# m4rch1n0/vqvae

Hardware: AMD Instinct MI355X
Metric: latents/sec through geodesic kNN+APSP+K-medoids (higher is better)
Workload: dtype f64-exact(u32 fixed point)

## Files before the change

vqvae_amd/csrc/common.hip:

```cpp
#include "geo_common.h"

#include <cstdlib>
#include <cstring>

namespace geo {

namespace {
struct OptionName { const char *name, *env; int Options::*field; };
const OptionName kOptionNames[] = {
    {"sssp_sb", "GEO_SSSP_SB", &Options::sssp_sb},
    {"sssp_act", "GEO_SSSP_ACT", &Options::sssp_act},
    {"sssp_sparse_div", "GEO_SSSP_SPARSE_DIV", &Options::sssp_sparse_div},
    {"sssp_map_div", "GEO_SSSP_MAP_DIV", &Options::sssp_map_div},
    {"sssp_group", "GEO_SSSP_GROUP", &Options::sssp_group},
    {"sssp_grouped_cap", "GEO_SSSP_GROUPED_CAP", &Options::sssp_grouped_cap},
    {"sssp_trace", "GEO_SSSP_TRACE", &Options::sssp_trace},
    {"sssp_u32", "GEO_SSSP_U32", &Options::sssp_u32},
    {"sssp_push", "GEO_SSSP_PUSH", &Options::sssp_push},
    {"sssp_order", "GEO_SSSP_ORDER", &Options::sssp_order},
    {"sssp_delta", "GEO_SSSP_DELTA", &Options::sssp_delta},
    {"sssp_push_blocks", "GEO_SSSP_PUSH_BLOCKS", &Options::sssp_push_blocks},
    {"knn_filter", "GEO_KNN_FILTER", &Options::knn_filter},
    {"kpp_grid", "GEO_KPP_GRID", &Options::kpp_grid},
    {"kpp_profile", "GEO_KPP_PROFILE", &Options::kpp_profile},
    {"jvp_mid", "GEO_JVP_MID", &Options::jvp_mid},
    {"jvp_back_valu", "GEO_JVP_BACK_VALU", &Options::jvp_back_valu},
    {"jvp_front_valu", "GEO_JVP_FRONT_VALU", &Options::jvp_front_valu},
    {"jvp_per_node", "GEO_JVP_PER_NODE", &Options::jvp_per_node},
    {"jvp_node_jacobian", "GEO_JVP_NODE_JACOBIAN", &Options::jvp_node_jacobian},
    {"jvp_start_dedup", "GEO_JVP_START_DEDUP", &Options::jvp_start_dedup},
    {"jvp_front_once", "GEO_JVP_FRONT_ONCE", &Options::jvp_front_once},
};
Options from_environment() {
    Options o;
    for (const OptionName &e : kOptionNames) {
        const char *v = getenv(e.env);
        if (!v) continue;
        if (e.field == &Options::jvp_mid) o.jvp_mid = v[0] == 'c' ? 2 : (v[0] == 'a' ? 3 : atoi(v));
        else o.*(e.field) = atoi(v);
    }
    return o;
}
}

Options &options() {
    static Options o = from_environment();
    return o;
}

static thread_local char g_err[512] = "";

void set_error(const char *fmt, ...) {
    va_list ap;
    va_start(ap, fmt);
    vsnprintf(g_err, sizeof(g_err), fmt, ap);
    va_end(ap);
}

constexpr int SCAN_THREADS = 256;
constexpr int SCAN_ITEMS = 8;
constexpr int SCAN_TILE = SCAN_THREADS * SCAN_ITEMS;

__global__ __launch_bounds__(SCAN_THREADS) void scan_tiles_kernel(const int32_t *__restrict__ in,
                                                                 int32_t *__restrict__ out,
                                                                 int32_t *__restrict__ tile_sums, int64_t n) {
    __shared__ int32_t wave_tot[SCAN_THREADS / 64];
    const int64_t base = (int64_t)blockIdx.x * SCAN_TILE + (int64_t)threadIdx.x * SCAN_ITEMS;
    int32_t v[SCAN_ITEMS];
    int32_t run = 0;
#pragma unroll
    for (int i = 0; i < SCAN_ITEMS; ++i) {
        int32_t x = (base + i < n) ? in[base + i] : 0;
        v[i] = run;
        run += x;
    }
    const int lane = threadIdx.x & 63, wave = threadIdx.x >> 6;
    int32_t inc = run;
#pragma unroll
    for (int off = 1; off < 64; off <<= 1) {
        int32_t t = __shfl_up(inc, off, 64);
        if (lane >= off) inc += t;
    }
    if (lane == 63) wave_tot[wave] = inc;
    __syncthreads();
    int32_t wave_base = 0, total = 0;
#pragma unroll
    for (int w = 0; w < SCAN_THREADS / 64; ++w) {
        if (w < wave) wave_base += wave_tot[w];
        total += wave_tot[w];
    }
    const int32_t excl = wave_base + inc - run;
#pragma unroll
    for (int i = 0; i < SCAN_ITEMS; ++i)
        if (base + i < n) out[base + i] = excl + v[i];
    if (threadIdx.x == 0) tile_sums[blockIdx.x] = total;
}

__global__ __launch_bounds__(SCAN_THREADS) void scan_add_kernel(int32_t *__restrict__ out,
                                                               const int32_t *__restrict__ tile_offs, int64_t n,
                                                               int64_t n_tiles) {
    const int64_t base = (int64_t)blockIdx.x * SCAN_TILE + (int64_t)threadIdx.x * SCAN_ITEMS;
    const int32_t add = tile_offs[blockIdx.x];
#pragma unroll
    for (int i = 0; i < SCAN_ITEMS; ++i)
        if (base + i < n) out[base + i] += add;
    if (blockIdx.x == 0 && threadIdx.x == 0) out[n] = tile_offs[n_tiles];
}

__global__ void scan_single_total_kernel(int32_t *out, const int32_t *tile_sums, int64_t n) {
    if (threadIdx.x == 0 && blockIdx.x == 0) out[n] = tile_sums[0];
}

static int64_t tiles_of(int64_t n) { return (n + SCAN_TILE - 1) / SCAN_TILE; }

size_t scan_tmp_bytes(int64_t n) {
    size_t total = 0;
    int64_t m = n;
    while (true) {
        int64_t t = tiles_of(m > 0 ? m : 1);
        total += align_up((size_t)(t + 1) * sizeof(int32_t)) * 2;
        if (t <= 1) break;
        m = t;
    }
    return total + 256;
}

static int scan_rec(const int32_t *in, int32_t *out, int64_t n, Arena &ar, hipStream_t s) {
    const int64_t t = tiles_of(n > 0 ? n : 1);
    int32_t *sums = ar.take<int32_t>((size_t)t + 1);
    int32_t *offs = ar.take<int32_t>((size_t)t + 1);
    if (!sums || !offs) {
        set_error("exclusive_scan: workspace too small");
        return GEO_E_WORKSPACE;
    }
    scan_tiles_kernel<<<dim3((unsigned)t), dim3(SCAN_THREADS), 0, s>>>(in, out, sums, n);
    GEO_LAUNCH_CHECK();
    if (t == 1) {
        scan_single_total_kernel<<<1, 64, 0, s>>>(out, sums, n);
        GEO_LAUNCH_CHECK();
        return GEO_OK;
    }
    int rc = scan_rec(sums, offs, t, ar, s);
    if (rc != GEO_OK) return rc;
    scan_add_kernel<<<dim3((unsigned)t), dim3(SCAN_THREADS), 0, s>>>(out, offs, n, t);
    GEO_LAUNCH_CHECK();
    return GEO_OK;
}

int exclusive_scan_i32(const int32_t *in, int32_t *out, int64_t n, void *tmp, size_t tmp_bytes,
                       int64_t *total_host, hipStream_t stream) {
    Arena ar(tmp, tmp_bytes);
    int rc = scan_rec(in, out, n, ar, stream);
    if (rc != GEO_OK) return rc;
    if (total_host) {
        int32_t tot = 0;
        GEO_HIP_CHECK(hipMemcpyAsync(&tot, out + n, sizeof(int32_t), hipMemcpyDeviceToHost, stream));
        GEO_HIP_CHECK(hipStreamSynchronize(stream));
        *total_host = tot;
    }
    return GEO_OK;
}

}

extern "C" int geo_version(void) { return 109; }
extern "C" const char *geo_last_error(void) { return geo::g_err; }

extern "C" int geo_set_option(const char *name, int32_t value) {
    if (name)
        for (const geo::OptionName &e : geo::kOptionNames)
            if (strcmp(name, e.name) == 0) {
                geo::options().*(e.field) = value;
                return GEO_OK;
            }
    geo::set_error("geo_set_option: unknown option '%s'", name ? name : "(null)");
    return GEO_E_ARG;
}
```

vqvae_amd/csrc/geo_common.h:

```cpp
#pragma once
#include <hip/hip_runtime.h>

#include <cstdarg>
#include <cstdint>
#include <cstdio>

#include "geo_hip.h"

namespace geo {

void set_error(const char *fmt, ...);

#define GEO_HIP_CHECK(expr)                                                                      \
    do {                                                                                         \
        hipError_t _e = (expr);                                                                  \
        if (_e != hipSuccess) {                                                                  \
            geo::set_error("%s failed: %s (%s:%d)", #expr, hipGetErrorString(_e), __FILE__, __LINE__); \
            return GEO_E_HIP;                                                                    \
        }                                                                                        \
    } while (0)

#define GEO_REQUIRE(cond, ...)              \
    do {                                    \
        if (!(cond)) {                      \
            geo::set_error(__VA_ARGS__);    \
            return GEO_E_ARG;               \
        }                                   \
    } while (0)

#define GEO_LAUNCH_CHECK() GEO_HIP_CHECK(hipGetLastError())

struct Options {
    int sssp_sb = -1, sssp_act = 1, sssp_sparse_div = -1, sssp_map_div = -1, sssp_group = 1, sssp_grouped_cap = 256,
        sssp_trace = 0, sssp_u32 = 1, sssp_push = 1 ,
        sssp_delta = 8 , sssp_order = 0 , sssp_push_blocks = 64, knn_filter = 1, kpp_grid = 256, kpp_profile = 0, jvp_mid = 0 ,
        jvp_back_valu = 0, jvp_front_valu = 0, jvp_per_node = 1 ,
        jvp_node_jacobian = 1 ,
        jvp_start_dedup = 1 ,
        jvp_front_once = 1 ;
};
Options &options();

static inline size_t align_up(size_t x, size_t a = 256) { return (x + a - 1) / a * a; }

struct Arena {
    char *base;
    size_t size, off;
    Arena(void *p, size_t n) : base(static_cast<char *>(p)), size(n), off(0) {}
    template <typename T>
    T *take(size_t count) {
        size_t bytes = align_up(count * sizeof(T));
        if (off + bytes > size) return nullptr;
        T *r = reinterpret_cast<T *>(base + off);
        off += bytes;
        return r;
    }
};

size_t scan_tmp_bytes(int64_t n);
int exclusive_scan_i32(const int32_t *in, int32_t *out, int64_t n, void *tmp, size_t tmp_bytes,
                       int64_t *total_host, hipStream_t stream);

static inline int grid_for(int64_t work_items, int per_block, int cap = 8192) {
    int64_t g = (work_items + per_block - 1) / per_block;
    if (g < 1) g = 1;
    if (g > cap) g = cap;
    return static_cast<int>(g);
}

}
```

vqvae_amd/csrc/jvp.hip:

```cpp
#include "geo_common.h"

#include <cmath>
#include <cstdlib>
#include <type_traits>
#include <vector>

namespace {

constexpr int TS = 32;
constexpr int NC = 128;
constexpr int MAX_BLOCKS = 4;
constexpr int FRONT_MAX_N1 = 1024;
constexpr int BACK_TS = 8;

typedef float f32x16 __attribute__((ext_vector_type(16)));
typedef __bf16 bf16x8 __attribute__((ext_vector_type(8)));
typedef unsigned short u16x8 __attribute__((ext_vector_type(8)));

struct Shape {
    int d, c0, c1, c2, co, s_out, pad3, p_out;
    int n1, n2;
    int opix_per_chunk, n_chunks;
};

// ... 1521 lines not shown
#pragma unroll
                for (int part = 0; part < 3; ++part) {
                    if (MODE != 1) *reinterpret_cast<u16x8 *>(&A3[part][0][ss][k0 + k8]) = pp[part];
                    if (MODE != 2) *reinterpret_cast<u16x8 *>(&A3[part][1][ss][k0 + k8]) = pt[part];
                }
            }
        }
        __syncthreads();
#pragma unroll
        for (int kq = 0; kq < 2; ++kq) {
            const int ks = wave * 2 + kq;
            bf16x8 ap[3], at[3];
#pragma unroll
            for (int part = 0; part < 3; ++part) {
                if (MODE != 1) ap[part] = *reinterpret_cast<const bf16x8 *>(&A3[part][0][r][ks * 16 + h * 8]);
                if (MODE != 2) at[part] = *reinterpret_cast<const bf16x8 *>(&A3[part][1][r][ks * 16 + h * 8]);
            }
#pragma unroll
            for (int nt = 0; nt < NT; ++nt) {
                bf16x8 b[3];
#pragma unroll
                for (int part = 0; part < 3; ++part)
                    b[part] = *reinterpret_cast<const bf16x8 *>(
                        W3b + ((((size_t)kb * 3 + part) * 8 + ks) * 2 + h) * (size_t)NP * 8 + (size_t)(nt * 32 + r) * 8);
                if (MODE != 1) accp[nt] = __builtin_amdgcn_mfma_f32_32x32x16_bf16(ap[2], b[0], accp[nt], 0, 0, 0);
                if (MODE != 2) acct[nt] = __builtin_amdgcn_mfma_f32_32x32x16_bf16(at[2], b[0], acct[nt], 0, 0, 0);
                if (MODE != 1) accp[nt] = __builtin_amdgcn_mfma_f32_32x32x16_bf16(ap[0], b[2], accp[nt], 0, 0, 0);
                if (MODE != 2) acct[nt] = __builtin_amdgcn_mfma_f32_32x32x16_bf16(at[0], b[2], acct[nt], 0, 0, 0);
                if (MODE != 1) accp[nt] = __builtin_amdgcn_mfma_f32_32x32x16_bf16(ap[1], b[1], accp[nt], 0, 0, 0);
                if (MODE != 2) acct[nt] = __builtin_amdgcn_mfma_f32_32x32x16_bf16(at[1], b[1], acct[nt], 0, 0, 0);
                if (MODE != 1) accp[nt] = __builtin_amdgcn_mfma_f32_32x32x16_bf16(ap[1], b[0], accp[nt], 0, 0, 0);
                if (MODE != 2) acct[nt] = __builtin_amdgcn_mfma_f32_32x32x16_bf16(at[1], b[0], acct[nt], 0, 0, 0);
                if (MODE != 1) accp[nt] = __builtin_amdgcn_mfma_f32_32x32x16_bf16(ap[0], b[1], accp[nt], 0, 0, 0);
                if (MODE != 2) acct[nt] = __builtin_amdgcn_mfma_f32_32x32x16_bf16(at[0], b[1], acct[nt], 0, 0, 0);
                if (MODE != 1) accp[nt] = __builtin_amdgcn_mfma_f32_32x32x16_bf16(ap[0], b[0], accp[nt], 0, 0, 0);
                if (MODE != 2) acct[nt] = __builtin_amdgcn_mfma_f32_32x32x16_bf16(at[0], b[0], acct[nt], 0, 0, 0);
            }
        }
    }
    float *red = reinterpret_cast<float *>(&A3[0][0][0][0]);
    const int row = threadIdx.x >> 3, c4 = (threadIdx.x & 7) * 4;
    const size_t nrow = MODE == 1 ? (row_map ? (size_t)row_map[slot0 + row] : node_of(row)) : slot0 + row;
    float *jrow = nullptr;
    if (MODE == 1 && jac_node) {
        const int64_t e = edge_of(row);
        if (e >= 0) jrow = jac_node + (nrow * unit_d + (size_t)(e % unit_d)) * NP;
    }
    double sumsq = 0.0;
#pragma unroll
    for (int nt = 0; nt < NT; ++nt) {
        __syncthreads();
#pragma unroll
        for (int q = 0; q < 16; ++q) {
            const int rr = (q & 3) + 8 * (q >> 2) + 4 * (lane >> 5);
            if (MODE != 1) red[((wave * 2 + 0) * 32 + rr) * 33 + (lane & 31)] = accp[nt][q];
            if (MODE != 2) red[((wave * 2 + 1) * 32 + rr) * 33 + (lane & 31)] = acct[nt][q];
        }
        __syncthreads();
#pragma unroll
        for (int c = 0; c < 4; ++c) {
            const int o = nt * 32 + c4 + c;
            if (o < P) {
                float x = b3[o / (s_out * s_out)], t = 0.f;
#pragma unroll
                for (int w = 0; w < 4; ++w) {
                    if (MODE != 1) x += red[((w * 2 + 0) * 32 + row) * 33 + c4 + c];
                    if (MODE != 2) t += red[((w * 2 + 1) * 32 + row) * 33 + c4 + c];
                }
                const float sg = MODE == 1 ? sg_node[nrow * NP + o] : 1.0f / (1.0f + expf(-x));
                if (MODE == 2) sg_node[nrow * NP + o] = sg;
                const float j = t * sg * (1.0f - sg);
                if (MODE == 1 && jrow) jrow[o] = j;
                sumsq += (double)(j * j);
            }
        }
    }
    sumsq += __shfl_xor(sumsq, 1, 64);
    sumsq += __shfl_xor(sumsq, 2, 64);
    sumsq += __shfl_xor(sumsq, 4, 64);
    if (MODE != 2 && (threadIdx.x & 7) == 0) norms[slot0 + row] = (float)sqrt(sumsq);
    }
}

__global__ __launch_bounds__(256) void combine_kernel(const float *__restrict__ norms, int64_t e_base, int64_t e_count,
                                                     int batch, int slots_per_group, float *__restrict__ len_out) {
    for (int64_t i = (int64_t)blockIdx.x * blockDim.x + threadIdx.x; i < e_count; i += (int64_t)gridDim.x * blockDim.x) {
        const int64_t chunk = i / batch, within = i % batch;
        const float a = norms[(chunk * 2 + 0) * slots_per_group + within];
        const float b = norms[(chunk * 2 + 1) * slots_per_group + within];
        len_out[e_base + i] = 0.5f * (a + b);
    }
}

__global__ __launch_bounds__(256) void pair_edges_kernel(int64_t n_nodes, int d, int64_t n_pseudo, int32_t *__restrict__ src,
                                                        int32_t *__restrict__ dst) {
    for (int64_t i = (int64_t)blockIdx.x * blockDim.x + threadIdx.x; i < n_pseudo; i += (int64_t)gridDim.x * blockDim.x) {
        const int64_t a = 2 * (i / d), b = a + 1 < n_nodes ? a + 1 : n_nodes - 1;
        src[i] = (int32_t)a;
        dst[i] = (int32_t)b;
    }
}

__global__ __launch_bounds__(256) void jacobian_lengths_kernel(const float *__restrict__ z, const int32_t *__restrict__ src,
                                                              const int32_t *__restrict__ dst, int64_t n_edges, int d, int p_out,
                                                              int np, const float *__restrict__ jac_node,
                                                              float *__restrict__ len_out) {
    const int64_t gid = (int64_t)blockIdx.x * 256 + threadIdx.x;
    const int l = (int)(gid & 15);
    int64_t e = gid >> 4;
    const bool live = e < n_edges;
    if (!live) e = n_edges - 1;
    const int64_t a = src[e], b = dst[e];
    float dz[16];
#pragma unroll
    for (int k = 0; k < 16; ++k) dz[k] = k < d ? z[b * d + k] - z[a * d + k] : 0.f;
    float end_norm[2];
#pragma unroll
    for (int side = 0; side < 2; ++side) {
        const float *J = jac_node + (size_t)(side ? b : a) * d * np;
        double sumsq = 0.0;
        for (int o = l; o < p_out; o += 16) {
            float v = 0.f;
#pragma unroll
            for (int k = 0; k < 16; ++k)
                if (k < d) v = fmaf(dz[k], J[(size_t)k * np + o], v);
            sumsq += (double)(v * v);
        }
        sumsq += __shfl_xor(sumsq, 1, 64);
        sumsq += __shfl_xor(sumsq, 2, 64);
        sumsq += __shfl_xor(sumsq, 4, 64);
        sumsq += __shfl_xor(sumsq, 8, 64);
        end_norm[side] = (float)sqrt(sumsq);
    }
    if (live && l == 0) len_out[e] = 0.5f * (end_norm[0] + end_norm[1]);
}

bool make_shape(const geo_decoder_desc *dc, Shape *s) {
    s->d = dc->latent_dim; s->c0 = dc->c0; s->c1 = dc->c1; s->c2 = dc->c2; s->co = dc->out_channels;
    if (dc->out_size == 28) { s->s_out = 4; s->pad3 = 3; }
    else if (dc->out_size == 32) { s->s_out = 8; s->pad3 = 1; }
    else return false;
    s->p_out = s->co * s->s_out * s->s_out;
    s->n1 = 4 * s->c1; s->n2 = 16 * s->c2;
    if (s->c2 <= 0 || NC % s->c2 != 0) return false;
    if (s->c1 <= 0 || 4 * s->c1 > FRONT_MAX_N1) return false;
    s->opix_per_chunk = NC / s->c2;
    if (s->opix_per_chunk > 16) s->opix_per_chunk = 16;
    s->n_chunks = 16 / s->opix_per_chunk;
    return true;
}

void make_chunks(const Shape &s, ChunkTable *t) {
    static const int order[16][2] = {{0, 1}, {0, 2}, {3, 1}, {3, 2}, {1, 0}, {2, 0}, {1, 3}, {2, 3},
                                     {1, 1}, {1, 2}, {2, 1}, {2, 2}, {0, 0}, {0, 3}, {3, 0}, {3, 3}};
    for (int ch = 0; ch < 16; ++ch) { t->nblk[ch] = 0; for (int i = 0; i < 16; ++i) t->opix[ch][i] = 0; }
    for (int ch = 0; ch < s.n_chunks; ++ch) {
        bool used[4] = {false, false, false, false};
        for (int lo = 0; lo < s.opix_per_chunk; ++lo) {
            const int oy = order[ch * s.opix_per_chunk + lo][0], ox = order[ch * s.opix_per_chunk + lo][1];
            t->opix[ch][lo] = oy * 4 + ox;
            for (int iy = 0; iy < 2; ++iy)
                for (int ix = 0; ix < 2; ++ix) {
                    const int ky = oy + 1 - 2 * iy, kx = ox + 1 - 2 * ix;
                    if (ky >= 0 && ky < 4 && kx >= 0 && kx < 4) used[iy * 2 + ix] = true;
                }
        }
        for (int ip = 0; ip < 4; ++ip)
            if (used[ip]) t->ipix[ch][t->nblk[ch]++] = ip;
    }
}

bool chunks_match_mid_geom(const ChunkTable &tab, int *bad_chunk) {
    for (int ch = 0; ch < 8; ++ch) {
        int nb = 0;
        bool ok = true;
        for (int ip = 0; ip < 4; ++ip) {
            const int blk = MidGeom::blk_of(ch, ip);
            if (blk >= 0) { ok = ok && tab.ipix[ch][blk] == ip; ++nb; }
        }
        ok = ok && nb == tab.nblk[ch] && tab.opix[ch][0] == MidGeom::opix(ch, 0) && tab.opix[ch][1] == MidGeom::opix(ch, 1);
        if (!ok) { *bad_chunk = ch; return false; }
    }
    return true;
}

struct Plan {
    Shape sh;
    int batch, tiles_per_group, slots_per_group;
    int64_t chunks_per_pass;
    size_t bytes;
    size_t pass_slots() const { return (size_t)chunks_per_pass * 2 * slots_per_group; }
};

constexpr int64_t MAX_SLOTS_PER_PASS = 1 << 20;

size_t round_up_to_tile(int64_t n) { return n > 0 ? ((size_t)n + TS - 1) / TS * TS : 0; }

size_t node_bytes(const Shape &s, int64_t n_nodes) {
    if (n_nodes <= 0) return 0;
    const size_t np = (size_t)((s.p_out + 31) / 32) * 32;
    return geo::align_up(round_up_to_tile(n_nodes) * s.n2 * 4) + geo::align_up(round_up_to_tile(n_nodes) * np * 4);
}

bool make_plan(const geo_decoder_desc *dc, int64_t n_edges, int batch, Plan *p) {
    if (!make_shape(dc, &p->sh)) return false;
    p->batch = batch;
    p->tiles_per_group = (batch + TS - 1) / TS;
    p->slots_per_group = p->tiles_per_group * TS;
    const int64_t chunks = (n_edges + batch - 1) / batch;
    int64_t cpp = MAX_SLOTS_PER_PASS / (2 * (int64_t)p->slots_per_group);
    if (cpp < 1) cpp = 1;
    if (cpp > chunks) cpp = chunks > 0 ? chunks : 1;
    p->chunks_per_pass = cpp;
    const Shape &s = p->sh;
    const size_t slots = p->pass_slots(), tiles = slots / TS, groups = (size_t)cpp * 2;
    size_t b = 0;
    b += geo::align_up((size_t)s.d * s.n1 * 4) + geo::align_up((size_t)s.n1 * 4);
    b += geo::align_up((size_t)s.n_chunks * MAX_BLOCKS * s.c1 * NC * 4);
    b += geo::align_up((size_t)s.n_chunks * MAX_BLOCKS * s.c1 * NC * 2 * 3);
    b += geo::align_up((size_t)16 * s.co * s.c2 * 4);
    b += geo::align_up((size_t)16 * s.c2 * 192 * 3 * 2);
    b += 2 * geo::align_up(slots * s.n1 * 4) + 2 * geo::align_up(slots * s.n2 * 4);
    b += geo::align_up(tiles * s.n1 * 4 * 8) + geo::align_up(tiles * s.n2 * 4 * 8);
    b += geo::align_up((groups + 1) * s.c1 * sizeof(NormConst)) + geo::align_up((groups + 1) * s.c2 * sizeof(NormConst));
    b += geo::align_up((groups + 1) * (size_t)(s.c1 > s.c2 ? s.c1 : s.c2) * sizeof(float2));
    b += geo::align_up(slots * 4) * 2;
    if (dc->norm == 2) b += 2 * geo::align_up(slots * 32 * sizeof(float4));
    p->bytes = b + 4096;
    return true;
}

enum { BACK_NODE_PRIMAL = 15 };

struct Route {
    int status = GEO_OK;
    char error[192] = "";
    Plan pl = {};
    int64_t run_edges = 0, passes = 0;
    bool batch_stats = false, track = false, group_norm = false;
    int front = GEO_JVP_FRONT_VALU, dmax = 16;
    int mid = GEO_JVP_MID_CHUNK, back = GEO_JVP_BACK_VALU;
    int back_nt = 0;
    int parts2 = 16;
    bool per_node = false, node_jacobian = false, dedup = false, front_once = false;
    size_t back_lds = 0;
    size_t jac_np = 0, jac_extra_bytes = 0;
    size_t bytes = 0;
};

bool route_error(Route *r, int status, const char *fmt, ...) {
    va_list ap;
    va_start(ap, fmt);
    vsnprintf(r->error, sizeof(r->error), fmt, ap);
    va_end(ap);
    r->status = status;
    return false;
}

bool make_route(const geo_decoder_desc *dc, const geo::Options &o, bool graph_edges, int64_t n_nodes, int64_t n_edges, int batch,
                const size_t *ws_bytes, Route *r) {
    *r = Route{};
    if (!dc) return route_error(r, GEO_E_ARG, "geo_decoder_jvp: null pointer");
    if (batch <= 0) return route_error(r, GEO_E_ARG, "geo_decoder_jvp: batch_size must be positive");
    Plan base;
    if (n_edges < 0 || n_nodes < 0 || !make_plan(dc, n_edges, batch, &base))
        return route_error(r, GEO_E_ARG, "geo_decoder_jvp: unsupported decoder (out_size %d, c2=%d must divide %d)", dc->out_size,
                           dc->c2, NC);
    const Shape &s = base.sh;

    r->batch_stats = dc->norm == 1 && dc->bn_train;
    r->track = r->batch_stats && dc->update_running && dc->rm1 && dc->rv1 && dc->rm2 && dc->rv2;
    r->group_norm = dc->norm == 2;
    r->dmax = s.d <= 16 ? 16 : (s.d <= 32 ? 32 : 64);
    r->front = s.d > 16 && s.n1 % 32 == 0 && o.jvp_front_valu == 0 ? GEO_JVP_FRONT_MFMA : GEO_JVP_FRONT_VALU;
    r->back_nt = (s.p_out + 31) / 32;
    const bool mid_all = s.c1 % 16 == 0 && s.c1 >= 32 && s.n_chunks == 8 && s.opix_per_chunk == 2 && o.jvp_mid != 2;
    const bool mid_pipe = mid_all && !r->group_norm && s.c1 == 128 && s.c2 == 64 && o.jvp_mid != 3;
    const bool back_mfma = s.c1 % 16 == 0 && s.c2 == 64 && (r->back_nt == 1 || r->back_nt == 6) && !o.jvp_back_valu;
    const bool per_node_kernels = graph_edges && !r->batch_stats && mid_all && back_mfma && o.jvp_per_node != 0;

    const size_t node_slots = round_up_to_tile(n_nodes);
    const size_t per_edge_end_bytes = base.bytes + (graph_edges ? node_bytes(s, n_nodes) : 0);
    Plan jpl;
    const int64_t n_pseudo = (n_nodes + 1) / 2 * s.d;
    size_t jac_bytes = 0;
    if (per_node_kernels && n_nodes > 0 && n_edges > 0 && s.d <= 16 && o.jvp_node_jacobian != 0 &&
        (o.jvp_node_jacobian != 1 || 4 * n_edges >= 3 * n_nodes * s.d) && n_pseudo < (int64_t)1 << 31 &&
        make_plan(dc, n_pseudo, batch, &jpl) && node_slots <= jpl.pass_slots()) {
        r->jac_np = (size_t)r->back_nt * 32;
        r->jac_extra_bytes = 2 * geo::align_up((size_t)n_pseudo * 4) + geo::align_up((size_t)n_nodes * s.d * r->jac_np * 4);
        jac_bytes = r->jac_extra_bytes + jpl.bytes + node_bytes(s, n_nodes);
    }
    r->bytes = jac_bytes > per_edge_end_bytes ? jac_bytes : per_edge_end_bytes;
    const size_t ws = ws_bytes ? *ws_bytes : r->bytes;
    r->node_jacobian = jac_bytes && ws >= jac_bytes;
    r->pl = r->node_jacobian ? jpl : base;
    r->run_edges = r->node_jacobian ? n_pseudo : n_edges;
    const int64_t chunks = (r->run_edges + batch - 1) / batch;
    r->passes = (chunks + r->pl.chunks_per_pass - 1) / r->pl.chunks_per_pass;
    const size_t run_ws = ws - (r->node_jacobian ? r->jac_extra_bytes : 0);
    r->per_node = per_node_kernels && node_slots && node_slots <= r->pl.pass_slots() &&
                  run_ws >= r->pl.bytes + node_bytes(s, n_nodes);
    const size_t slots = r->pl.pass_slots(), tiles = slots / TS, groups = (size_t)r->pl.chunks_per_pass * 2;
    r->dedup = r->batch_stats && graph_edges && mid_pipe && back_mfma && o.jvp_start_dedup != 0 &&
               (2 * slots + groups) * 4 <= tiles * s.n1 * 4 * 8 && (size_t)r->back_nt * 32 <= (size_t)s.n1;
    r->front_once = r->dedup && r->front == GEO_JVP_FRONT_VALU && o.jvp_front_once != 0 && s.n1 == FRONT_EDGE_N1 &&
                    tiles * s.c1 * 4 * 8 + (2 * slots + groups) * 4 <= tiles * s.n1 * 4 * 8 &&
                    (size_t)base.slots_per_group * s.n1 * 4 < ((size_t)1 << 31);

    r->mid = r->per_node ? GEO_JVP_MID_ALL_TANGENT
           : mid_pipe    ? (r->dedup ? GEO_JVP_MID_PIPE_DEDUP : GEO_JVP_MID_PIPE)
           : mid_all     ? GEO_JVP_MID_ALL
                         : GEO_JVP_MID_CHUNK;
    r->parts2 = mid_pipe && !r->per_node ? 4 : (mid_all ? 1 : 16);
    r->back = r->dedup ? GEO_JVP_BACK_DEDUP : r->per_node ? GEO_JVP_BACK_PER_NODE : back_mfma ? GEO_JVP_BACK_MFMA : GEO_JVP_BACK_VALU;
    r->back_lds = ((size_t)2 * BACK_TS * 16 * (s.c2 + 4) + (size_t)16 * s.co * (s.c2 + 4) + (size_t)BACK_TS * s.p_out) * 4;

    if (!(s.d >= 1 && s.d <= 64)) return route_error(r, GEO_E_ARG, "geo_decoder_jvp: latent_dim %d not in [1,64]", s.d);
    if (!(s.c1 == 128 || s.c1 == 64 || s.c1 == 32))
        return route_error(r, GEO_E_ARG, "geo_decoder_jvp: dec_channels[1]=%d not in {32,64,128}", s.c1);
    if (!(dc->norm >= 0 && dc->norm <= 2)) return route_error(r, GEO_E_ARG, "geo_decoder_jvp: unknown norm code %d", dc->norm);
    if (s.c2 % 16 != 0) return route_error(r, GEO_E_ARG, "geo_decoder_jvp: dec_channels[2]=%d must be a multiple of 16", s.c2);
    if (r->back_lds > 160 * 1024)
        return route_error(r, GEO_E_ARG, "geo_decoder_jvp: decoder too wide for the back kernel (%zu B LDS)", r->back_lds);
    if (run_ws < r->pl.bytes) return route_error(r, GEO_E_WORKSPACE, "geo_decoder_jvp: workspace %zu < %zu", run_ws, r->pl.bytes);
    if (r->group_norm && !(dc->groups1 == 32 && dc->groups2 == 32 && s.c2 == 64 && back_mfma && mid_all))
        return route_error(r, GEO_E_ARG,
                           "geo_decoder_jvp: GroupNorm needs 32 groups per layer and dec_channels[2] == 64 (got %d/%d groups, c2=%d)",
                           dc->groups1, dc->groups2, s.c2);
    return true;
}

int encode_route(const Route &r) {
    const int64_t passes = r.passes < 0x7fff ? r.passes : 0x7fff;
    return r.front | (r.dmax == 16 ? 0 : (r.dmax == 32 ? 1 : 2)) << 2 | r.mid << 4 | r.back << 8 |
           (r.per_node ? GEO_JVP_PER_NODE : 0) | (r.node_jacobian ? GEO_JVP_NODE_JACOBIAN : 0) | (r.dedup ? GEO_JVP_DEDUP : 0) |
           (r.front_once ? GEO_JVP_FRONT_ONCE : 0) | (int)passes << 16;
}

struct Buffers {
    float *M01, *b01, *B2p, *W3p, *pre1, *tpre1, *pre2, *tpre2, *norms;
    unsigned short *B3, *W3b;
    double *part1, *part2; NormConst *k1, *k2;
    float2 *stats;
    int32_t *slot_valid;
    float4 *gs1, *gs2;
    float *pre2_node, *sg_node;
    int32_t *row_map, *rep, *n_compact;
    float *sg_compact, *jac;
    ChunkTable tab;
};

struct Pass {
    int mid, back;
    int64_t tiles, e_base, n_edges;
    int tiles_per_group, batch, unit_d, stat;
    const float *z, *z_start, *z_end;
    const int32_t *src, *dst;
    float *mid_pre2;
    const float *back_pre2;
    int64_t slots() const { return tiles * TS; }
    int64_t groups() const { return tiles / tiles_per_group; }
};

template <int... Vs, class F>
void pick_int(int v, F &&f) { ((v == Vs ? (void)f(std::integral_constant<int, Vs>{}) : (void)0), ...); }
template <class F>
void pick_bool(bool v, F &&f) { if (v) f(std::true_type{}); else f(std::false_type{}); }

int cu_count(int *n) {
    static int n_cu = 0;
    if (n_cu == 0) {
        int devid = 0, cus = 0;
        GEO_HIP_CHECK(hipGetDevice(&devid));
        GEO_HIP_CHECK(hipDeviceGetAttribute(&cus, hipDeviceAttributeMultiprocessorCount, devid));
        n_cu = cus > 0 ? cus : 256;
    }
    *n = n_cu;
    return GEO_OK;
}

int launch_start_runs(const Pass &p, const Buffers &b, hipStream_t stream) {
    start_runs_kernel<<<(unsigned)(p.groups() / 2), 256, 0, stream>>>(p.src, p.e_base, p.n_edges, p.batch, p.tiles_per_group * TS,
                                                                     b.row_map, b.rep, b.n_compact);
    GEO_LAUNCH_CHECK();
    return GEO_OK;
}

int launch_front(const Route &r, const Pass &p, const Buffers &b, hipStream_t stream) {
    const Shape &s = r.pl.sh;
    if (r.front_once)
// ... 30 lines not shown
                b.stats, (int)p.groups(), C, dc->momentum, const_cast<float *>(l1 ? dc->rm1 : dc->rm2),
                const_cast<float *>(l1 ? dc->rv1 : dc->rv2));
        GEO_LAUNCH_CHECK();
    }
    if (r.group_norm) {
        const int32_t *prim_row = nullptr;
        if (!l1 && p.back == GEO_JVP_BACK_PER_NODE) {
            slot_node_kernel<<<geo::grid_for(p.slots(), 256), 256, 0, stream>>>(p.src, p.dst, p.e_base, p.n_edges, p.batch,
                                                                                p.tiles_per_group, p.slots(), b.slot_valid);
            prim_row = b.slot_valid;
        }
        group_stats_kernel<<<geo::grid_for(p.slots() * 32, 256), 256, 0, stream>>>(
            l1 ? b.pre1 : p.back_pre2, l1 ? b.tpre1 : b.tpre2, p.slots(), npx, C, 32, dc->eps, l1 ? b.gs1 : b.gs2, prim_row);
        GEO_LAUNCH_CHECK();
    }
    return GEO_OK;
}

int launch_mid(const Route &r, const geo_decoder_desc *dc, const Pass &p, const Buffers &b, hipStream_t stream) {
    const Shape &s = r.pl.sh;
    if (p.mid == GEO_JVP_MID_PIPE || p.mid == GEO_JVP_MID_PIPE_DEDUP) {
        const bool dedup = p.mid == GEO_JVP_MID_PIPE_DEDUP;
        const int64_t chunks = p.groups() / 2;
        if (dedup && !r.front_once)
            if (const int rc = launch_start_runs(p, b, stream)) return rc;
        int n_cu = 0;
        if (const int rc = cu_count(&n_cu)) return rc;
        const int64_t pipe_tiles = dedup ? p.tiles / 2 : p.tiles;
        const unsigned grid = (unsigned)std::min<int64_t>(pipe_tiles, n_cu);
        pick_bool(dedup, [&](auto end_only) {
            mid_pipe_kernel<decltype(end_only)::value><<<grid, 512, 0, stream>>>(
                b.pre1, b.tpre1, b.k1, p.stat, p.tiles_per_group, (int)pipe_tiles, s.c2, b.B3, dc->b2, p.mid_pre2, b.tpre2, b.part2,
                p.stat, p.e_base, p.n_edges, p.batch);
        });
        GEO_LAUNCH_CHECK();
        if (dedup) {
            mid_start_kernel<false><<<dim3(1, (unsigned)chunks), 512, 0, stream>>>(
                b.pre1, b.tpre1, b.k1, p.tiles_per_group, b.B3, dc->b2, p.mid_pre2, b.tpre2, b.part2, b.row_map, b.rep, b.n_compact,
                p.e_base, p.n_edges, p.batch);
            GEO_LAUNCH_CHECK();
            pick_bool(r.front_once, [&](auto once) {
                mid_start_kernel<true, decltype(once)::value>
                    <<<dim3((unsigned)((p.tiles_per_group + 1) / 2), (unsigned)chunks), 512, 0, stream>>>(
                        b.pre1, b.tpre1, b.k1, p.tiles_per_group, b.B3, dc->b2, p.mid_pre2, b.tpre2, b.part2, b.row_map, b.rep,
                        b.n_compact, p.e_base, p.n_edges, p.batch);
            });
            GEO_LAUNCH_CHECK();
        }
    } else if (p.mid == GEO_JVP_MID_ALL || p.mid == GEO_JVP_MID_ALL_TANGENT) {
        pick_int<128, 64, 32>(s.c1, [&](auto c1) {
            pick_bool(r.group_norm, [&](auto gn) {
                pick_bool(p.mid == GEO_JVP_MID_ALL_TANGENT, [&](auto tangent_only) {
                    mid_all_kernel<decltype(c1)::value, decltype(gn)::value, decltype(tangent_only)::value>
                        <<<(unsigned)p.tiles, 512, 0, stream>>>(b.pre1, b.tpre1, b.k1, p.stat, p.tiles_per_group, s.c2, b.B3, dc->b2,
                                                                p.mid_pre2, b.tpre2, b.part2, p.stat, b.slot_valid, b.gs1, p.e_base,
                                                                p.n_edges, p.batch);
                });
            });
        });
        GEO_LAUNCH_CHECK();
    } else {
        pick_int<128, 64, 32>(s.c1, [&](auto c1) {
            mid_bf16_kernel<decltype(c1)::value><<<dim3((unsigned)p.tiles, (unsigned)s.n_chunks), 256, 0, stream>>>(
                b.pre1, b.tpre1, b.k1, p.stat, p.tiles_per_group, b.tab, s.opix_per_chunk, s.c2, b.B3, dc->b2, p.mid_pre2, b.tpre2,
                b.part2, p.stat, b.slot_valid);
        });
        GEO_LAUNCH_CHECK();
    }
    return GEO_OK;
}

int launch_back(const Route &r, const geo_decoder_desc *dc, const Pass &p, const Buffers &b, hipStream_t stream) {
    const Shape &s = r.pl.sh;
    if (p.back == GEO_JVP_BACK_VALU) {
        back_kernel<<<(unsigned)(p.slots() / BACK_TS), 256, r.back_lds, stream>>>(
            p.back_pre2, b.tpre2, b.k2, p.stat, p.tiles_per_group * TS, s.c2, s.co, s.s_out, s.pad3, b.W3p, dc->b3, b.norms);
        GEO_LAUNCH_CHECK();
        return GEO_OK;
    }
    const unsigned tiles = (unsigned)p.tiles, side_tiles = (unsigned)(p.tiles / 2), chunks = (unsigned)(p.groups() / 2);
    pick_int<1, 6>(r.back_nt, [&](auto nt) {
        constexpr int NT = decltype(nt)::value;
        if (p.back == GEO_JVP_BACK_DEDUP) {
            back_mfma_kernel<NT, false, 0><<<side_tiles, 256, 0, stream>>>(
                p.back_pre2, b.tpre2, b.k2, 1, p.tiles_per_group, s.co, s.s_out, b.W3b, dc->b3, b.norms, nullptr, nullptr, nullptr,
                nullptr, 0, 0, 1, nullptr, 0, nullptr, nullptr, 2);
            back_mfma_kernel<NT, false, 2><<<chunks, 256, 0, stream>>>(
                p.back_pre2, b.tpre2, b.k2, 1, p.tiles_per_group, s.co, s.s_out, b.W3b, dc->b3, b.norms, nullptr, b.sg_compact, nullptr,
                nullptr, 0, 0, 1, nullptr, 0, nullptr, b.n_compact, 1);
            back_mfma_kernel<NT, false, 1><<<side_tiles, 256, 0, stream>>>(
                p.back_pre2, b.tpre2, b.k2, 1, p.tiles_per_group, s.co, s.s_out, b.W3b, dc->b3, b.norms, nullptr, b.sg_compact, nullptr,
                nullptr, 0, 0, 1, nullptr, 0, b.row_map, nullptr, 1);
            return;
        }
        pick_bool(r.group_norm, [&](auto gn) {
            constexpr bool GN = decltype(gn)::value;
            if (p.back == GEO_JVP_BACK_MFMA)
                back_mfma_kernel<NT, GN, 0><<<tiles, 256, 0, stream>>>(p.back_pre2, b.tpre2, b.k2, p.stat, p.tiles_per_group, s.co,
                                                                      s.s_out, b.W3b, dc->b3, b.norms, b.gs2);
            else if (p.back == GEO_JVP_BACK_PER_NODE)
                back_mfma_kernel<NT, GN, 1><<<tiles, 256, 0, stream>>>(p.back_pre2, b.tpre2, b.k2, 0, p.tiles_per_group, s.co, s.s_out,
                                                                      b.W3b, dc->b3, b.norms, b.gs2, b.sg_node, p.src, p.dst, p.e_base,
                                                                      p.n_edges, p.batch, b.jac, p.unit_d);
            else
                back_mfma_kernel<NT, GN, 2><<<tiles, 256, 0, stream>>>(p.back_pre2, b.tpre2, b.k2, 0, p.tiles_per_group, s.co, s.s_out,
                                                                      b.W3b, dc->b3, b.norms, b.gs2, b.sg_node);
        });
    });
    GEO_LAUNCH_CHECK();
    return GEO_OK;
}

int launch_pass(const Route &r, const geo_decoder_desc *dc, const Pass &p, const Buffers &b, hipStream_t stream) {
    if (r.front_once)
        if (const int rc = launch_start_runs(p, b, stream)) return rc;
    if (const int rc = launch_front(r, p, b, stream)) return rc;
    if (const int rc = launch_stats(r, dc, 1, p, b, stream)) return rc;
    if (const int rc = launch_mid(r, dc, p, b, stream)) return rc;
    if (const int rc = launch_stats(r, dc, 2, p, b, stream)) return rc;
    return launch_back(r, dc, p, b, stream);
}

int run_jvp(const geo_decoder_desc *dc, const Route &r, const float *z, int64_t n_nodes, const int32_t *src, const int32_t *dst,
            const float *z_start, const float *z_end, int64_t n_edges, float *len_out, void *ws, size_t ws_bytes,
            hipStream_t stream) {
    const Plan &pl = r.pl;
    const Shape &s = pl.sh;
    const int batch = pl.batch;
    const size_t slots = pl.pass_slots(), tiles = slots / TS, groups = (size_t)pl.chunks_per_pass * 2;

    geo::Arena ar(ws, ws_bytes);
    Buffers b = {};
    int32_t *psrc = nullptr, *pdst = nullptr;
    if (r.node_jacobian) {
        psrc = ar.take<int32_t>((size_t)r.run_edges);
        pdst = ar.take<int32_t>((size_t)r.run_edges);
        b.jac = ar.take<float>((size_t)n_nodes * s.d * r.jac_np);
        GEO_REQUIRE(b.jac != nullptr, "geo_decoder_jvp_edges: workspace carve failed");
    }
    b.M01 = ar.take<float>((size_t)s.d * s.n1);
    b.b01 = ar.take<float>((size_t)s.n1);
    b.B2p = ar.take<float>((size_t)s.n_chunks * MAX_BLOCKS * s.c1 * NC);
    b.B3 = ar.take<unsigned short>((size_t)s.n_chunks * MAX_BLOCKS * s.c1 * NC * 3);
    b.W3p = ar.take<float>((size_t)16 * s.co * s.c2);
    b.W3b = ar.take<unsigned short>((size_t)16 * s.c2 * 192 * 3);
    b.pre1 = ar.take<float>(slots * s.n1); b.tpre1 = ar.take<float>(slots * s.n1);
    b.pre2 = ar.take<float>(slots * s.n2); b.tpre2 = ar.take<float>(slots * s.n2);
    b.part1 = ar.take<double>(tiles * s.n1 * 4); b.part2 = ar.take<double>(tiles * s.n2 * 4);
    b.k1 = ar.take<NormConst>((groups + 1) * s.c1); b.k2 = ar.take<NormConst>((groups + 1) * s.c2);
    b.norms = ar.take<float>(slots);
    b.stats = ar.take<float2>((groups + 1) * (size_t)(s.c1 > s.c2 ? s.c1 : s.c2));
    b.slot_valid = ar.take<int32_t>(slots);
    if (r.group_norm) { b.gs1 = ar.take<float4>(slots * 32); b.gs2 = ar.take<float4>(slots * 32); }
    const size_t node_slots = round_up_to_tile(n_nodes);
    if (r.per_node) {
        b.pre2_node = ar.take<float>(node_slots * s.n2);
        b.sg_node = ar.take<float>(node_slots * (size_t)((s.p_out + 31) / 32) * 32);
    }
    GEO_REQUIRE(b.slot_valid && (!r.group_norm || b.gs2) && (!r.per_node || b.sg_node), "geo_decoder_jvp: workspace carve failed");
    if (r.dedup) {
        b.row_map = reinterpret_cast<int32_t *>(b.part1 + (r.front_once ? tiles * s.c1 * 4 : 0)); b.rep = b.row_map + slots; b.n_compact = b.rep + slots;
        b.sg_compact = b.pre1;
    }

    make_chunks(s, &b.tab);
    int bad_chunk = 0;
// ... 135 lines not shown
```

Measured before the change: 2.391 million.

## Add streaming dedup back kernel with register double-buffered prefetch across tiles

Adds a specialised back-stage kernel for the dedup path (C2=64, NT=1, no group norm). Each workgroup walks several consecutive tiles and prefetches the next pre2/tpre2 slice into registers while the current one is normalised and fed through split-bf16 MFMAs. It replaces the per-tile back_mfma launches for the end and start sides and is on by default through a new option. The aim is to hide global load latency and amortise setup such as bias and norm constants across tiles, at the cost of more registers and hard-coded shape assumptions.

```diff
diff --git a/vqvae_amd/csrc/common.hip b/vqvae_amd/csrc/common.hip
--- a/vqvae_amd/csrc/common.hip
+++ b/vqvae_amd/csrc/common.hip
@@ -30,6 +30,7 @@
     {"jvp_node_jacobian", "GEO_JVP_NODE_JACOBIAN", &Options::jvp_node_jacobian},
     {"jvp_start_dedup", "GEO_JVP_START_DEDUP", &Options::jvp_start_dedup},
     {"jvp_front_once", "GEO_JVP_FRONT_ONCE", &Options::jvp_front_once},
+    {"jvp_back_stream", "GEO_JVP_BACK_STREAM", &Options::jvp_back_stream},
 };
 Options from_environment() {
     Options o;
@@ -163,7 +164,7 @@
 
 }
 
-extern "C" int geo_version(void) { return 109; }
+extern "C" int geo_version(void) { return 110; }
 extern "C" const char *geo_last_error(void) { return geo::g_err; }
 
 extern "C" int geo_set_option(const char *name, int32_t value) {
diff --git a/vqvae_amd/csrc/geo_common.h b/vqvae_amd/csrc/geo_common.h
--- a/vqvae_amd/csrc/geo_common.h
+++ b/vqvae_amd/csrc/geo_common.h
@@ -37,7 +37,8 @@
         jvp_back_valu = 0, jvp_front_valu = 0, jvp_per_node = 1 ,
         jvp_node_jacobian = 1 ,
         jvp_start_dedup = 1 ,
-        jvp_front_once = 1 ;
+        jvp_front_once = 1 ,
+        jvp_back_stream = 1 ;
 };
 Options &options();
 
diff --git a/vqvae_amd/csrc/jvp.hip b/vqvae_amd/csrc/jvp.hip
--- a/vqvae_amd/csrc/jvp.hip
+++ b/vqvae_amd/csrc/jvp.hip
@@ -1627,6 +1627,159 @@
     }
 }
 
+constexpr int BACK_STREAM_MAX_TILES = 4;
+constexpr int BACK_STREAM_TILES = 4;  static_assert(BACK_STREAM_TILES <= BACK_STREAM_MAX_TILES);
+template <bool START>
+__global__ __launch_bounds__(256, 2) void back_stream_kernel(const float *__restrict__ pre2, const float *__restrict__ tpre2,
+                                                         const NormConst *__restrict__ consts2, int tiles_per_group,
+                                                         int tiles_per_wg, int co_n, int s_out,
+                                                         const unsigned short *__restrict__ W3b, const float *__restrict__ b3,
+                                                         float *__restrict__ norms, const float *__restrict__ sg_node,
+                                                         const int32_t *__restrict__ row_map) {
+    constexpr int C2 = 64, KB = 128, LDK = KB + 8, NP = 32, N2 = 16 * C2;
+    __shared__ __attribute__((aligned(16))) unsigned short A3[3][2][TS][LDK];
+    __shared__ NormConst kc[C2];
+    __shared__ int32_t rows[START ? BACK_STREAM_MAX_TILES * TS : 1];
+    const int ranges = (tiles_per_group + tiles_per_wg - 1) / tiles_per_wg;
+    const int group = ((int)blockIdx.x / ranges) * 2 + (START ? 0 : 1);
+    const int t_first = ((int)blockIdx.x % ranges) * tiles_per_wg;
+    const int t_end = t_first + tiles_per_wg < tiles_per_group ? t_first + tiles_per_wg : tiles_per_group;
+    const int lane = threadIdx.x & 63, wave = threadIdx.x >> 6;
+    const int P = co_n * s_out * s_out;
+    const int r = lane & 31, h = lane >> 5;
+    const int ss = threadIdx.x >> 3, k0 = (threadIdx.x & 7) * 16, cb = k0 & (C2 - 1);
+    const int c4 = (threadIdx.x & 7) * 4;
+    float bias[4];
+#pragma unroll
+    for (int c = 0; c < 4; ++c) bias[c] = c4 + c < P ? b3[(c4 + c) / (s_out * s_out)] : 0.f;
+    for (int c = threadIdx.x; c < C2; c += 256) kc[c] = consts2[(size_t)group * C2 + c];
+
+    size_t slot0 = ((size_t)group * tiles_per_group + t_first) * TS;
+    size_t prow = START ? (size_t)row_map[slot0 + ss] : slot0 + ss;
+    if (START && (int)threadIdx.x < (t_end - t_first) * TS) rows[threadIdx.x] = row_map[slot0 + threadIdx.x];
+    const float *xp = pre2 + prow * N2 + k0, *xt = tpre2 + (slot0 + ss) * N2 + k0;
+    float4 rp[2][4], rt[2][4];
+    auto request = [&](auto buf, const float *p, const float *t) {
+        constexpr int B = decltype(buf)::value;
+#pragma unroll
+        for (int i = 0; i < 4; ++i) {
+            rp[B][i] = *reinterpret_cast<const float4 *>(p + 4 * i);
+            rt[B][i] = *reinterpret_cast<const float4 *>(t + 4 * i);
+        }
+    };
+    auto comp = [](const float4 &v, int i) { return i == 0 ? v.x : i == 1 ? v.y : i == 2 ? v.z : v.w; };
+    request(std::integral_constant<int, 0>{}, xp, xt);
+
+    for (int tile = t_first; tile < t_end; ++tile) {
+        const bool more = tile + 1 < t_end;
+        auto next_row = [&]() { return START ? (size_t)rows[(more ? tile + 1 - t_first : 0) * TS + ss] : slot0 + TS + ss; };
+        const float4 sgv = START ? *reinterpret_cast<const float4 *>(sg_node + prow * NP + c4) : make_float4(0.f, 0.f, 0.f, 0.f);
+        f32x16 accp, acct;
+#pragma unroll
+        for (int i = 0; i < 16; ++i) { accp[i] = 0.f; acct[i] = 0.f; }
+
+        auto block = [&](auto buf, int kb) {
+            constexpr int B = decltype(buf)::value;
+            bf16x8 bw[2][3];
+#pragma unroll
+            for (int kq = 0; kq < 2; ++kq)
+#pragma unroll
+                for (int part = 0; part < 3; ++part)
+                    bw[kq][part] = *reinterpret_cast<const bf16x8 *>(
+                        W3b + ((((size_t)kb * 3 + part) * 8 + wave * 2 + kq) * 2 + h) * (size_t)NP * 8 + (size_t)r * 8);
+            __builtin_amdgcn_sched_barrier(0);
+            const bool wrap = B == 1 && kb == 7;
+            const int kn = wrap && !more ? 7 : kb + 1;
+            request(std::integral_constant<int, 1 - B>{}, wrap && more ? pre2 + next_row() * N2 + k0 : xp + kn * KB,
+                    wrap && more ? xt + (size_t)TS * N2 : xt + kn * KB);
+            __builtin_amdgcn_sched_barrier(0);
+            __syncthreads();
+#pragma unroll
+            for (int k8 = 0; k8 < 16; k8 += 8) {
+                unsigned wp[3][4], wt[3][4];
+#pragma unroll
+                for (int k = 0; k < 8; k += 2) {
+                    float a0, a1, t0, t1;
+                    norm_relu(kc[cb + k8 + k], comp(rp[B][(k8 + k) >> 2], k & 3), comp(rt[B][(k8 + k) >> 2], k & 3), &a0, &t0);
+                    norm_relu(kc[cb + k8 + k + 1], comp(rp[B][(k8 + k) >> 2], (k & 3) + 1), comp(rt[B][(k8 + k) >> 2], (k & 3) + 1), &a1, &t1);
+                    if (!START) split3_pair(a0, a1, wp[0][k >> 1], wp[1][k >> 1], wp[2][k >> 1]);
+                    split3_pair(t0, t1, wt[0][k >> 1], wt[1][k >> 1], wt[2][k >> 1]);
+                }
+#pragma unroll
+                for (int part = 0; part < 3; ++part) {
+                    if (!START)
+                        *reinterpret_cast<uint4 *>(&A3[part][0][ss][k0 + k8]) = make_uint4(wp[part][0], wp[part][1], wp[part][2], wp[part][3]);
+                    *reinterpret_cast<uint4 *>(&A3[part][1][ss][k0 + k8]) = make_uint4(wt[part][0], wt[part][1], wt[part][2], wt[part][3]);
+                }
+            }
+            __syncthreads();
+#pragma unroll
+            for (int kq = 0; kq < 2; ++kq) {
+                const int ks = wave * 2 + kq;
+                bf16x8 ap[3], at[3];
+#pragma unroll
+                for (int part = 0; part < 3; ++part) {
+                    if (!START) ap[part] = *reinterpret_cast<const bf16x8 *>(&A3[part][0][r][ks * 16 + h * 8]);
+                    at[part] = *reinterpret_cast<const bf16x8 *>(&A3[part][1][r][ks * 16 + h * 8]);
+                }
+                const bf16x8 *b = bw[kq];
+                if (!START) accp = __builtin_amdgcn_mfma_f32_32x32x16_bf16(ap[2], b[0], accp, 0, 0, 0);
+                acct = __builtin_amdgcn_mfma_f32_32x32x16_bf16(at[2], b[0], acct, 0, 0, 0);
+                if (!START) accp = __builtin_amdgcn_mfma_f32_32x32x16_bf16(ap[0], b[2], accp, 0, 0, 0);
+                acct = __builtin_amdgcn_mfma_f32_32x32x16_bf16(at[0], b[2], acct, 0, 0, 0);
+                if (!START) accp = __builtin_amdgcn_mfma_f32_32x32x16_bf16(ap[1], b[1], accp, 0, 0, 0);
+                acct = __builtin_amdgcn_mfma_f32_32x32x16_bf16(at[1], b[1], acct, 0, 0, 0);
+                if (!START) accp = __builtin_amdgcn_mfma_f32_32x32x16_bf16(ap[1], b[0], accp, 0, 0, 0);
+                acct = __builtin_amdgcn_mfma_f32_32x32x16_bf16(at[1], b[0], acct, 0, 0, 0);
+                if (!START) accp = __builtin_amdgcn_mfma_f32_32x32x16_bf16(ap[0], b[1], accp, 0, 0, 0);
+                acct = __builtin_amdgcn_mfma_f32_32x32x16_bf16(at[0], b[1], acct, 0, 0, 0);
+                if (!START) accp = __builtin_amdgcn_mfma_f32_32x32x16_bf16(ap[0], b[0], accp, 0, 0, 0);
+                acct = __builtin_amdgcn_mfma_f32_32x32x16_bf16(at[0], b[0], acct, 0, 0, 0);
+            }
+        };
+#pragma unroll 1
+        for (int kb = 0; kb < 8; kb += 2) {
+            block(std::integral_constant<int, 0>{}, kb);
+            block(std::integral_constant<int, 1>{}, kb + 1);
+        }
+
+        float *red = reinterpret_cast<float *>(&A3[0][0][0][0]);
+        __syncthreads();
+#pragma unroll
+        for (int q = 0; q < 16; ++q) {
+            const int rr = (q & 3) + 8 * (q >> 2) + 4 * (lane >> 5);
+            if (!START) red[((wave * 2 + 0) * 32 + rr) * 33 + (lane & 31)] = accp[q];
+            red[((wave * 2 + 1) * 32 + rr) * 33 + (lane & 31)] = acct[q];
+        }
+        __syncthreads();
+        double sumsq = 0.0;
+#pragma unroll
+        for (int c = 0; c < 4; ++c) {
+            const int o = c4 + c;
+            if (o < P) {
+                float x = bias[c], t = 0.f;
+#pragma unroll
+                for (int w = 0; w < 4; ++w) {
+                    if (!START) x += red[((w * 2 + 0) * 32 + ss) * 33 + c4 + c];
+                    t += red[((w * 2 + 1) * 32 + ss) * 33 + c4 + c];
+                }
+                const float sg = START ? comp(sgv, c) : 1.0f / (1.0f + expf(-x));
+                const float j = t * sg * (1.0f - sg);
+                sumsq += (double)(j * j);
+            }
+        }
+        sumsq += __shfl_xor(sumsq, 1, 64);
+        sumsq += __shfl_xor(sumsq, 2, 64);
+        sumsq += __shfl_xor(sumsq, 4, 64);
+        if ((threadIdx.x & 7) == 0) norms[slot0 + ss] = (float)sqrt(sumsq);
+
+        if (more) prow = next_row();
+        slot0 += TS;
+        xp = pre2 + prow * N2 + k0;
+        xt += (size_t)TS * N2;
+    }
+}
+
 __global__ __launch_bounds__(256) void combine_kernel(const float *__restrict__ norms, int64_t e_base, int64_t e_count,
                                                      int batch, int slots_per_group, float *__restrict__ len_out) {
     for (int64_t i = (int64_t)blockIdx.x * blockDim.x + threadIdx.x; i < e_count; i += (int64_t)gridDim.x * blockDim.x) {
@@ -1787,7 +1940,7 @@
     int mid = GEO_JVP_MID_CHUNK, back = GEO_JVP_BACK_VALU;
     int back_nt = 0;
     int parts2 = 16;
-    bool per_node = false, node_jacobian = false, dedup = false, front_once = false;
+    bool per_node = false, node_jacobian = false, dedup = false, front_once = false, back_stream = false;
     size_t back_lds = 0;
     size_t jac_np = 0, jac_extra_bytes = 0;
     size_t bytes = 0;
@@ -1852,6 +2005,7 @@
     r->front_once = r->dedup && r->front == GEO_JVP_FRONT_VALU && o.jvp_front_once != 0 && s.n1 == FRONT_EDGE_N1 &&
                     tiles * s.c1 * 4 * 8 + (2 * slots + groups) * 4 <= tiles * s.n1 * 4 * 8 &&
                     (size_t)base.slots_per_group * s.n1 * 4 < ((size_t)1 << 31);
+    r->back_stream = r->dedup && r->back_nt == 1 && !r->group_norm && o.jvp_back_stream != 0;
 
     r->mid = r->per_node ? GEO_JVP_MID_ALL_TANGENT
            : mid_pipe    ? (r->dedup ? GEO_JVP_MID_PIPE_DEDUP : GEO_JVP_MID_PIPE)
@@ -2048,6 +2202,18 @@
     pick_int<1, 6>(r.back_nt, [&](auto nt) {
         constexpr int NT = decltype(nt)::value;
         if (p.back == GEO_JVP_BACK_DEDUP) {
+            if constexpr (NT == 1)
+                if (r.back_stream) {
+                    const unsigned grid = chunks * (unsigned)((p.tiles_per_group + BACK_STREAM_TILES - 1) / BACK_STREAM_TILES);
+                    back_stream_kernel<false><<<grid, 256, 0, stream>>>(p.back_pre2, b.tpre2, b.k2, p.tiles_per_group, BACK_STREAM_TILES,
+                                                                        s.co, s.s_out, b.W3b, dc->b3, b.norms, nullptr, nullptr);
+                    back_mfma_kernel<NT, false, 2><<<chunks, 256, 0, stream>>>(
+                        p.back_pre2, b.tpre2, b.k2, 1, p.tiles_per_group, s.co, s.s_out, b.W3b, dc->b3, b.norms, nullptr, b.sg_compact,
+                        nullptr, nullptr, 0, 0, 1, nullptr, 0, nullptr, b.n_compact, 1);
+                    back_stream_kernel<true><<<grid, 256, 0, stream>>>(p.back_pre2, b.tpre2, b.k2, p.tiles_per_group, BACK_STREAM_TILES,
+                                                                       s.co, s.s_out, b.W3b, dc->b3, b.norms, b.sg_compact, b.row_map);
+                    return;
+                }
             back_mfma_kernel<NT, false, 0><<<side_tiles, 256, 0, stream>>>(
                 p.back_pre2, b.tpre2, b.k2, 1, p.tiles_per_group, s.co, s.s_out, b.W3b, dc->b3, b.norms, nullptr, nullptr, nullptr,
                 nullptr, 0, 0, 1, nullptr, 0, nullptr, nullptr, 2);
```

Result: no change. 2.413 million, median of 4 (+0.9%).
